# joaobuibergen/roms-trunk-mgh

Hardware: AMD Instinct MI355X
Metric: simulated-days/wall-sec (higher is better)
Workload: dtype f64; 1 GPU; BENCHMARK3 2048x256x30 NT=2 nonlinear 3-D step incl. 59 step2d calls, U3/C4 tracer advection, analytic atmospheric forcing, bulk fluxes + KPP + diagnostics every step; tiling=1x1, halo_transport=none, rccl_ranks=0, graph_exchanges=1, ndtfast=20, finite=True

## Files before the change

### include/roms_hip.h

```cpp
#ifndef ROMS_HIP_H
#define ROMS_HIP_H

#ifdef __cplusplus
extern "C" {
#endif

enum roms_kind {
  K_2D = 0, K_2D_T2, K_2D_T3, K_2D_NT,
  K_3DR, K_3DW, K_3DR_T2, K_3DW_T2, K_3DW_NAT, K_4DT, K_3DR_NT, K_3DW_T3
};

enum roms_field_id {
#define ROMS_FIELD(name, kind, owner) FID_##name,
#include "roms_fields.def"
#undef ROMS_FIELD
  FID_COUNT
};

typedef struct roms_fields {
#define ROMS_FIELD(name, kind, owner) double *name;
#include "roms_fields.def"
#undef ROMS_FIELD
} roms_fields_t;

// ... 127 lines not shown
int roms_hip_set_diagnostics(int nDIA, int ntsDIA, int ntstart, int nrrec);
int roms_hip_set_diags(const roms_step_idx_t *s);
int roms_hip_get_diagnostic(int dia_id, int itrc, int accumulated, double *host, long n_doubles);
int roms_hip_dia_index(int dia_id, int hdif, int rotated);
int roms_hip_set_floats(int Nfloats, const int *Ftype, const double *Tinfo, const double *Fz0,
                        const double *xcoord, const double *ycoord);
int roms_hip_floats_put(const double *track, long n_track, const int *bounded, long n_bounded);
int roms_hip_floats_get(double *track, long n_track, int *bounded, long n_bounded);
int roms_hip_step_floats(const roms_step_idx_t *s, double time, const int nfl[5]);
int roms_hip_set_tides(int NTC, int MTC, const double *Tperiod, const double *SSH_Tamp, const double *SSH_Tphase,
                       const double *UV_Tangle, const double *UV_Tphase, const double *UV_Tmajor, const double *UV_Tminor,
                       const double *angler, double tide_start, int ramp_tides, double dstart,
                       int add_fsobc, const double *zeta_base, int add_m2obc, const double *ubar_base,
                       const double *vbar_base);
int roms_hip_tides(double time);
int roms_hip_wvelocity(const roms_step_idx_t *s);
int roms_hip_diag(const roms_step_idx_t *s, double *out12);

int roms_hip_step2d_loop(roms_step_idx_t *s, int *indx1);

int roms_hip_graph_exchanges(int on);
int roms_hip_graph_exchanges_state(void);

int roms_hip_exchange(int field_id, int level);

typedef struct { int peer; int tag; long count; double *buf; } roms_halo_msg_t;
typedef int (*roms_halo_relay_fn)(void *user, int nsend, const roms_halo_msg_t *send,
                                  int nrecv, const roms_halo_msg_t *recv);
int roms_hip_set_halo_relay(roms_halo_relay_fn fn, void *user);
int roms_hip_halo_plan(const roms_bounds_t *b, int rank, int *out);

int roms_hip_timing_enable(int on);
double roms_hip_timing_last_ms(const char *entry);

int roms_hip_calib_stream(long n_doubles);

int roms_hip_check_guards(void);

#ifdef __cplusplus
}
#endif
#endif
```

### roms_trunk_mgh_amd/csrc/capi.hip

```cpp
#include "roms_dev.h"
#include <algorithm>
#include <map>
#include <vector>

RomsCtx g_ctx;

static const int k_field_kind[FID_COUNT] = {
#define ROMS_FIELD(name, kind, owner) kind,
#include "roms_fields.def"
#undef ROMS_FIELD
};
static const char *k_field_name[FID_COUNT] = {
#define ROMS_FIELD(name, kind, owner) #name,
#include "roms_fields.def"
#undef ROMS_FIELD
};

int roms_fail(const char *where, const char *what)
{
  g_ctx.last_error = std::string(where) + ": " + what;
  return 8;
}

long roms_field_count(int kind, const roms_bounds_t &b)
// ... 216 lines not shown
    (void)hipStreamDestroy(g_ctx.stream);
    g_ctx.stream = nullptr;
    g_ctx.devc = nullptr;
    return roms_fail("roms_hip_init", "hipMalloc of the constant block failed");
  }
  memset(&g_ctx.hostc, 0, sizeof(RomsDev));
  g_ctx.devc_dirty = true;
  g_ctx.inited = true;
  g_ctx.loopback = false;
  if (g_ctx.have_nccl_id) {
    if (ntileI * ntileJ == 1 && rank != 0) { roms_hip_finalize(); return roms_fail("roms_hip_init", "one tile: rank must be 0"); }
    int rc = halo_init();
    if (rc) { roms_hip_finalize(); return rc; }
    g_ctx.loopback = ntileI * ntileJ == 1;
  }
  return 0;
}

extern "C" int roms_hip_finalize(void)
{
  if (!g_ctx.inited) return 0;
  (void)hipStreamSynchronize(g_ctx.stream);
  (void)roms_hip_graph_exchanges(0);
  roms_rowm_release();
  snapshot_release();
  halo_finalize();
  diag_release();
  for (int i = 0; i < FID_COUNT; i++) {
    guarded_free(&g_ctx.dev[i], &g_ctx.dev_base[i]);
    g_ctx.host[i] = nullptr;
    g_ctx.count[i] = 0;
  }
  for (int q = 0; q < ROMS_NWS3; q++) guarded_free(&g_ctx.hostc.ws3[q], &g_ctx.ws3_base[q]);
  for (int q = 0; q < 32; q++) guarded_free(&g_ctx.hostc.ws2[q], &g_ctx.ws2_base[q]);
  sources_release();
  clima_release();
  avg_release();
  floats_release();
  tides_release();
  dia_release();
  if (g_ctx.devc) (void)hipFree(g_ctx.devc);
  g_ctx.devc = nullptr;
  if (g_ctx.stream) (void)hipStreamDestroy(g_ctx.stream);
  g_ctx.stream = nullptr;
  g_ctx.inited = false;
  g_ctx.have_bounds = g_ctx.have_params = false;
// ... 509 lines not shown
```

### roms_trunk_mgh_amd/csrc/halo.hip

```cpp
#include "roms_dev.h"
#include <dlfcn.h>
#include <vector>

typedef struct { char internal[128]; } rccl_uid_t;
typedef void *rccl_comm_t;
typedef int (*fn_getuid)(rccl_uid_t *);
typedef int (*fn_initrank)(rccl_comm_t *, int, rccl_uid_t, int);
typedef int (*fn_destroy)(rccl_comm_t);
typedef int (*fn_send)(const void *, size_t, int, int, rccl_comm_t, hipStream_t);
typedef int (*fn_recv)(void *, size_t, int, int, rccl_comm_t, hipStream_t);
typedef int (*fn_group)(void);
typedef int (*fn_allreduce)(const void *, void *, size_t, int, int, rccl_comm_t, hipStream_t);
typedef const char *(*fn_errstr)(int);
static struct {
  bool loaded = false;
  fn_getuid getuid = nullptr;
  fn_initrank initrank = nullptr;
  fn_destroy destroy = nullptr;
  fn_send send = nullptr;
  fn_recv recv = nullptr;
  fn_group gstart = nullptr, gend = nullptr;
  fn_allreduce allreduce = nullptr;
  fn_errstr errstr = nullptr;
} rccl;
// ... 133 lines not shown
  const int Lm = b.Lm;
  double *P = A + (long)k * nij;
  for (int m = 1; m <= b.NghostPoints; m++) P[I2(Lm + m, j)] = P[I2(m, j)];
  for (int m = 0; m <= 2; m++) P[I2(-m, j)] = P[I2(Lm - m, j)];
}

struct PeriodicArgs {
  double *A[8];
  int koff[8], jmin[8], jmax[8];
  int n, nktot, jlo;
};
__global__ void k_periodic_multi(const RomsDev *__restrict__ c, PeriodicArgs a)
{
  DEV_PROLOGUE(c)
  const int j = a.jlo + blockIdx.x * blockDim.x + threadIdx.x;
  const int kk = blockIdx.y;
  int f = 0;
  while (f + 1 < a.n && kk >= a.koff[f + 1]) f++;
  if (kk >= a.nktot || j < a.jmin[f] || j > a.jmax[f]) return;
  const int Lm = b.Lm;
  double *P = a.A[f] + (long)(kk - a.koff[f]) * nij;
  for (int m = 1; m <= b.NghostPoints; m++) P[I2(Lm + m, j)] = P[I2(m, j)];
  for (int m = 0; m <= 2; m++) P[I2(-m, j)] = P[I2(Lm - m, j)];
}

#define HALO_MAX_ITEMS 8
#define HALO_MAX_MSGS 8
struct PackArgs {
  double *A[HALO_MAX_ITEMS];
  int koff[HALO_MAX_ITEMS];
  int n, nktot, nmsg, unpack;
  int i0[HALO_MAX_MSGS], j0[HALO_MAX_MSGS], wi[HALO_MAX_MSGS], wj[HALO_MAX_MSGS];
  long off[HALO_MAX_MSGS];
  double *buf;
  int LBi, LBj;
  long ni, nij;
};
__global__ void k_pack_multi(const RomsDev *__restrict__, PackArgs a)
{
  const int LBi = a.LBi, LBj = a.LBj;
  const long ni = a.ni, nij = a.nij;
  const int m = blockIdx.z;
  const int wi = a.wi[m], cnt = wi * a.wj[m];
  const int r = blockIdx.x * blockDim.x + threadIdx.x;
  const int kk = blockIdx.y;
  if (r >= cnt) return;
// ... 72 lines not shown
    out[q++] = x.peer; out[q++] = x.tag; out[q++] = x.i0; out[q++] = x.wi; out[q++] = x.j0; out[q++] = x.wj;
  }
  for (int m = 0; m < p.nrecv; m++) {
    const HaloMsg &x = p.recv[m];
    out[q++] = x.peer; out[q++] = x.tag; out[q++] = x.i0; out[q++] = x.wi; out[q++] = x.j0; out[q++] = x.wj;
  }
  return 0;
}

static void ensure_neigh();

bool halo_rccl_capturable() { return g_ctx.nccl_comm != nullptr && g_relay == nullptr; }
int halo_reserve_buffers()
{
  ensure_neigh();
  if (!g_have_plan) { g_plan = make_plan(g_ctx.b, g_neigh); g_have_plan = true; }
  long smax = 0, rmax = 0;
  for (int m = 0; m < g_plan.nsend; m++) smax += (long)g_plan.send[m].wi * g_plan.send[m].wj;
  for (int m = 0; m < g_plan.nrecv; m++) rmax += (long)g_plan.recv[m].wi * g_plan.recv[m].wj;
  const long planes = (long)HALO_MAX_ITEMS * (g_ctx.b.N + 1);
  return ensure_buffers((size_t)((smax > rmax ? smax : rmax) * planes));
}

struct HaloItem { int gtype, nk; double *A; };

static int exchange_all(const HaloItem *items, int nitems)
{
  if (!g_have_plan) { g_plan = make_plan(g_ctx.b, g_neigh); g_have_plan = true; }
  const HaloPlan &pl = g_plan;
  if (pl.nsend == 0 && pl.nrecv == 0) return 0;
  long nktot = 0;
  for (int f = 0; f < nitems; f++) nktot += items[f].nk;
  PackArgs pa;
  pa.n = nitems; pa.nktot = (int)nktot;
  pa.LBi = g_ctx.b.LBi; pa.LBj = g_ctx.b.LBj;
  pa.ni = g_ctx.b.UBi - g_ctx.b.LBi + 1;
  pa.nij = pa.ni * (long)(g_ctx.b.UBj - g_ctx.b.LBj + 1);
  {
    int koff = 0;
    for (int f = 0; f < nitems; f++) { pa.A[f] = items[f].A; pa.koff[f] = koff; koff += items[f].nk; }
  }
  long soff[HALO_MAX_MSGS], roff[HALO_MAX_MSGS], stot = 0, rtot = 0;
  int smax = 1, rmax = 1;
  for (int m = 0; m < pl.nsend; m++) {
    soff[m] = stot;
    const int cnt = pl.send[m].wi * pl.send[m].wj;
    stot += nktot * cnt;
// ... 59 lines not shown
  return 0;
}

static void ensure_neigh()
{
  const roms_bounds_t &b = g_ctx.b;
  if (!g_have_neigh) {
    int v[12];
    roms_hip_tile_neighbors(g_ctx.rank, b.ntileI, b.ntileJ, b.NghostPoints, b.NghostPoints,
                            b.EWperiodic, b.NSperiodic, v);
    g_neigh = Neigh{v[0], v[1], v[2], v[3], v[4], v[5], v[6], v[7], v[8], v[9], v[10], v[11]};
    if (g_ctx.loopback && b.EWperiodic) {
      g_neigh.Wtile = g_neigh.Etile = g_ctx.rank;
      if (b.NghostPoints != 3) g_neigh.GrecvW = g_neigh.GsendE = b.NghostPoints + 1;
    }
    g_have_neigh = true;
  }
}

static int halo_run(const HaloItem *items, int nitems)
{
  const roms_bounds_t &b = g_ctx.b;
  if (nitems <= 0) return 0;
  if (b.ntileI * b.ntileJ == 1 && !g_ctx.loopback) {
    if (!b.EWperiodic) return 0;
    for (int f0 = 0; f0 < nitems; f0 += HALO_MAX_ITEMS) {
      PeriodicArgs pa;
      pa.n = nitems - f0 < HALO_MAX_ITEMS ? nitems - f0 : HALO_MAX_ITEMS;
      int nktot = 0, jlo = b.UBj, jhi = b.LBj;
      for (int f = 0; f < pa.n; f++) {
        const HaloItem &it = items[f0 + f];
        int jmin, jmax;
        if (b.NSperiodic) { jmin = b.Jstr; jmax = b.Jend; }
        else { jmin = (it.gtype == GT_R || it.gtype == GT_U) ? b.JstrR : b.Jstr; jmax = b.JendR; }
        pa.A[f] = it.A; pa.koff[f] = nktot; pa.jmin[f] = jmin; pa.jmax[f] = jmax;
        nktot += it.nk;
        jlo = jmin < jlo ? jmin : jlo;
        jhi = jmax > jhi ? jmax : jhi;
      }
      pa.nktot = nktot; pa.jlo = jlo;
      dim3 grid((jhi - jlo + 1 + 63) / 64, nktot);
      hipLaunchKernelGGL(k_periodic_multi, grid, dim3(64), 0, g_ctx.stream, g_ctx.devc, pa);
    }
    KERNEL_CHECK("k_periodic_multi");
    return 0;
  }
// ... 4 lines not shown
      hipLaunchKernelGGL(k_periodic_ew, grid, dim3(64), 0, g_ctx.stream, g_ctx.devc, items[f].A, items[f].nk, b.LBj, b.UBj);
    }
    KERNEL_CHECK("k_periodic_ew");
  }
  for (int f0 = 0; f0 < nitems; f0 += HALO_MAX_ITEMS) {
    const int n = nitems - f0 < HALO_MAX_ITEMS ? nitems - f0 : HALO_MAX_ITEMS;
    const int rc = exchange_all(items + f0, n);
    if (rc) return rc;
  }
  return 0;
}

static std::vector<HaloItem> g_batch;
static bool g_batching = false;
void halo_batch_begin() { g_batching = true; g_batch.clear(); }
int halo_batch_end()
{
  g_batching = false;
  const int rc = halo_run(g_batch.data(), (int)g_batch.size());
  g_batch.clear();
  return rc;
}

int halo_exchange3d(int gtype, int nk, double *A)
{
  const HaloItem it{gtype, nk, A};
  if (g_batching) { g_batch.push_back(it); return 0; }
  return halo_run(&it, 1);
}

int halo_exchange2d(int gtype, double *A, int) { return halo_exchange3d(gtype, 1, A); }

static double *g_coll = nullptr;
static size_t g_coll_doubles = 0;
static void coll_release()
{
  if (g_coll) (void)hipHostFree(g_coll);
  g_coll = nullptr;
  g_coll_doubles = 0;
}
int halo_allreduce_sum(double *A, long n)
{
  if (n <= 0) return 0;
  const int world = g_ctx.ntileI * g_ctx.ntileJ, me = g_ctx.rank;
  if (g_ctx.nccl_comm) {
    if (!rccl.allreduce) return roms_fail("collect", "RCCL symbol ncclAllReduce missing");
    RCCL_TRY(rccl.allreduce(A, A, (size_t)n, RCCL_FLOAT64, RCCL_SUM, (rccl_comm_t)g_ctx.nccl_comm, g_ctx.stream));
    return 0;
  }
// ... 45 lines not shown
```

### roms_trunk_mgh_amd/csrc/k_base.hip

```cpp
#include "roms_dev.h"

int roms_entry_check(const char *name);

int lbc_code(const roms_params_t &p, int sd, int v)
{
  if (p.lbc[sd][v]) return p.lbc[sd][v];
  return sd == LBS_WEST ? p.lbc_west : sd == LBS_EAST ? p.lbc_east : sd == LBS_SOUTH ? p.lbc_south : p.lbc_north;
}

int check_lbc()
{
  const roms_bounds_t &b = g_ctx.b;
  const roms_params_t &p = g_ctx.p;
  if (b.NSperiodic)
    return roms_fail("check_lbc", "N-S periodic grids are not implemented on this path");
  for (int sd = LBS_WEST; sd <= LBS_NORTH; sd++) {
    const bool periodic = (sd <= LBS_EAST) ? b.EWperiodic != 0 : b.NSperiodic != 0;
    for (int v = 0; v < LBV_COUNT; v++) {
      const int c = lbc_code(p, sd, v);
      if (periodic) {
        if (c != LBC_PERIODIC) return roms_fail("check_lbc", "a periodic direction needs LBC = Per on both of its sides");
        continue;
      }
      bool ok = c == LBC_CLOSED || c == LBC_GRADIENT || c == LBC_CLAMPED || c == LBC_RADIATION || c == LBC_RADIATION_NUDGING;
// ... 371 lines not shown
  a.T = g_ctx.dev[FID_vbar] + (long)(know - 1) * nij_host();
  a.ssh_only = g_ctx.hostc.tides.ssh_only;
  bc_acquire(a);
  a.dt2d = dt2d;
  return edge_bc(a);
}
int bc_v2d(int kout, const roms_step_idx_t *s)
{
  BcArgs a = bc_args(LBV_VBAR, g_ctx.dev[FID_vbar] + (long)(kout - 1) * nij_host(), 1);
  int know = kout; double dt2d = 0.0;
  if (s) bc_know(s, &know, &dt2d);
  else if (needs_know(a)) return roms_fail("bc_v2d", "this condition needs the barotropic time indices");
  a.Xold = g_ctx.dev[FID_vbar] + (long)(know - 1) * nij_host();
  a.D = g_ctx.dev[FID_vbar_bry];
  a.Zn = g_ctx.dev[FID_zeta] + (long)(kout - 1) * nij_host();
  a.Z = g_ctx.dev[FID_zeta] + (long)(know - 1) * nij_host();
  a.Zb = g_ctx.dev[FID_zeta_bry];
  a.T = g_ctx.dev[FID_ubar] + (long)(know - 1) * nij_host();
  a.ssh_only = g_ctx.hostc.tides.ssh_only;
  bc_acquire(a);
  a.dt2d = dt2d;
  return edge_bc(a);
}
int bc_u3d(int nout, int nstp)
{
  const long n3r = nij_host() * g_ctx.b.N;
  BcArgs a = bc_args(LBV_U, g_ctx.dev[FID_u] + (long)(nout - 1) * n3r, g_ctx.b.N);
  a.Xold = g_ctx.dev[FID_u] + (long)(nstp - 1) * n3r;
  a.D = g_ctx.dev[FID_u_bry];
  return edge_bc(a);
}
int bc_v3d(int nout, int nstp)
{
  const long n3r = nij_host() * g_ctx.b.N;
  BcArgs a = bc_args(LBV_V, g_ctx.dev[FID_v] + (long)(nout - 1) * n3r, g_ctx.b.N);
  a.Xold = g_ctx.dev[FID_v] + (long)(nstp - 1) * n3r;
  a.D = g_ctx.dev[FID_v_bry];
  return edge_bc(a);
}
int bc_t3d(int nout, int itrc, int nstp)
{
  const long n3r = nij_host() * g_ctx.b.N;
  BcArgs a = bc_args(LBV_T, g_ctx.dev[FID_t] + ((long)(nout - 1) + 3L * (itrc - 1)) * n3r, g_ctx.b.N);
  a.Xold = g_ctx.dev[FID_t] + ((long)(nstp - 1) + 3L * (itrc - 1)) * n3r;
  a.D = g_ctx.dev[FID_t_bry] + (long)(itrc - 1) * n3r;
  const int ic = g_ctx.hostc.clima.ic[itrc - 1];
  if (ic > 0) a.C = g_ctx.hostc.clima.Tnudgcof + (long)(ic - 1) * n3r;
  return edge_bc(a);
}
int bc_w3d(double *A)
{
  int rc = edge_bc(bc_args(-1, A, g_ctx.b.N + 1));
  if (rc) return rc;
  return halo_exchange3d(GT_R, g_ctx.b.N + 1, A);
}

__global__ void __launch_bounds__(BLK_X *BLK_Y)
k_set_massflux(const RomsDev *__restrict__ c, int nrhs)
{
  DEV_PROLOGUE(c)
  const Blk XB = xcd_block();
  const int i = b.IstrT + XB.x * BLK_X + threadIdx.x;
  const int j = b.JstrT + XB.y * BLK_Y + threadIdx.y;
  const int k = XB.z + 1;
  if (i > b.IendT || j > b.JendT) return;
  const gcd_t Hz = (gcd_t)(c->F.Hz);
  const gcd_t u = (gcd_t)(c->F.u + (long)(nrhs - 1) * n3r);
  const gcd_t v = (gcd_t)(c->F.v + (long)(nrhs - 1) * n3r);
  const double hz = Hz[I3(i, j, k)];
  if (i >= b.IstrP)
    GF(Huon)[I3(i, j, k)] = 0.5 * (hz + Hz[I3(i - 1, j, k)]) * u[I3(i, j, k)] * GF(on_u)[I2(i, j)];
  if (j >= b.JstrP)
    GF(Hvom)[I3(i, j, k)] = 0.5 * (hz + Hz[I3(i, j - 1, k)]) * v[I3(i, j, k)] * GF(om_v)[I2(i, j)];
}

extern "C" int roms_hip_set_massflux(const roms_step_idx_t *s)
{
  int rc = roms_entry_check("roms_hip_set_massflux");
  if (rc) return rc;
  ScopedTimer tm("set_massflux");
  const roms_bounds_t &b = g_ctx.b;
  dim3 grid = grid2d(b.IendT - b.IstrT + 1, b.JendT - b.JstrT + 1);
  grid.z = b.N;
  hipLaunchKernelGGL(k_set_massflux, grid, block2d(), 0, g_ctx.stream, g_ctx.devc, s->nrhs);
  KERNEL_CHECK("k_set_massflux");
  halo_batch_begin();
  halo_exchange3d(GT_U, b.N, g_ctx.dev[FID_Huon]);
  halo_exchange3d(GT_V, b.N, g_ctx.dev[FID_Hvom]);
  return halo_batch_end();
}

template <int NMAX>
__global__ void __launch_bounds__(BLK_X *BLK_Y)
k_omega(const RomsDev *__restrict__ c)
{
  DEV_PROLOGUE(c)
  const Blk XB = xcd_block();
  const int i = b.Istr + XB.x * BLK_X + threadIdx.x;
  const int j = b.Jstr + XB.y * BLK_Y + threadIdx.y;
  if (i > b.Iend || j > b.Jend) return;
  const gcd_t Huon = (gcd_t)(c->F.Huon);
  const gcd_t Hvom = (gcd_t)(c->F.Hvom);
  const gcd_t z_w = (gcd_t)(c->F.z_w);
  const gd_t W = (gd_t)(c->F.W);
  double w[NMAX + 1];
  w[0] = 0.0;
#pragma unroll
  for (int k = 1; k <= NMAX; k++) {
    if (k <= N) {
      w[k] = w[k - 1] - (Huon[I3(i + 1, j, k)] - Huon[I3(i, j, k)] +
                         Hvom[I3(i, j + 1, k)] - Hvom[I3(i, j, k)]);
    }
  }
  const double zw0 = z_w[I3W(i, j, 0)];
  double wN = 0.0;
#pragma unroll
  for (int k = 1; k <= NMAX; k++) if (k == N) wN = w[k];
  const double wrk = wN / (z_w[I3W(i, j, N)] - zw0);
  W[I3W(i, j, 0)] = 0.0;
#pragma unroll
  for (int k = 1; k <= NMAX; k++) {
    if (k < N) W[I3W(i, j, k)] = w[k] - wrk * (z_w[I3W(i, j, k)] - zw0);
  }
  W[I3W(i, j, N)] = 0.0;
}

__global__ void k_src_omega(const RomsDev *__restrict__ c)
{
  DEV_PROLOGUE(c)
  const int is = blockIdx.x * blockDim.x + threadIdx.x;
  if (is >= c->src.n || c->src.D[is] != 2) return;
  const int i = c->src.I[is], j = c->src.J[is];
  if (i < b.Istr || i > b.Iend || j < b.Jstr || j > b.Jend) return;
  if (c->src.wmap[I2(i, j)] != is + 1) return;
  const double *__restrict__ Huon = c->F.Huon, *__restrict__ Hvom = c->F.Hvom, *__restrict__ z_w = c->F.z_w;
  double *__restrict__ W = c->F.W;
  double w = 0.0;
  for (int k = 1; k <= N; k++) {
    w = w - (Huon[I3(i + 1, j, k)] - Huon[I3(i, j, k)] + Hvom[I3(i, j + 1, k)] - Hvom[I3(i, j, k)]) +
        c->src.Qsrc[is + (long)c->src.n * (k - 1)];
    W[I3W(i, j, k)] = w;
  }
  const double zw0 = z_w[I3W(i, j, 0)];
  const double wrk = w / (z_w[I3W(i, j, N)] - zw0);
  for (int k = N - 1; k >= 1; k--) W[I3W(i, j, k)] = W[I3W(i, j, k)] - wrk * (z_w[I3W(i, j, k)] - zw0);
  W[I3W(i, j, N)] = 0.0;
}

extern "C" int roms_hip_omega(const roms_step_idx_t *s)
{
  (void)s;
  int rc = roms_entry_check("roms_hip_omega");
  if (rc) return rc;
  if ((rc = check_lbc())) return rc;
  ScopedTimer tm("omega");
  const roms_bounds_t &b = g_ctx.b;
  dim3 grid = grid2d(b.Iend - b.Istr + 1, b.Jend - b.Jstr + 1);
  if (b.N <= 16) hipLaunchKernelGGL(k_omega<16>, grid, block2d(), 0, g_ctx.stream, g_ctx.devc);
  else if (b.N <= 32) hipLaunchKernelGGL(k_omega<32>, grid, block2d(), 0, g_ctx.stream, g_ctx.devc);
  else hipLaunchKernelGGL(k_omega<ROMS_MAXN>, grid, block2d(), 0, g_ctx.stream, g_ctx.devc);
  KERNEL_CHECK("k_omega");
  if ((g_ctx.p.point_sources & 2) && g_ctx.hostc.src.n > 0) {
    hipLaunchKernelGGL(k_src_omega, dim3((g_ctx.hostc.src.n + 63) / 64), dim3(64), 0, g_ctx.stream, g_ctx.devc);
    KERNEL_CHECK("k_src_omega");
  }
  return bc_w3d(g_ctx.dev[FID_W]);
}

__global__ void k_set_zeta(const RomsDev *__restrict__ c)
{
  DEV_PROLOGUE(c)
  const Blk XB = xcd_block();
  const int i = b.IstrR + XB.x * BLK_X + threadIdx.x;
  const int j = b.JstrR + XB.y * BLK_Y + threadIdx.y;
  if (i > b.IendR || j > b.JendR) return;
  const double z = GF(Zt_avg1)[I2(i, j)];
  GF(zeta)[I2(i, j)] = z;
  GF(zeta)[I2(i, j) + nij] = z;
}

extern "C" int roms_hip_set_zeta(const roms_step_idx_t *s)
{
  (void)s;
  int rc = roms_entry_check("roms_hip_set_zeta");
  if (rc) return rc;
  ScopedTimer tm("set_zeta");
  const roms_bounds_t &b = g_ctx.b;
  hipLaunchKernelGGL(k_set_zeta, grid2d(b.IendR - b.IstrR + 1, b.JendR - b.JstrR + 1), block2d(), 0,
                     g_ctx.stream, g_ctx.devc);
  KERNEL_CHECK("k_set_zeta");
  return halo_exchange3d(GT_R, 2, g_ctx.dev[FID_zeta]);
}

__global__ void __launch_bounds__(BLK_X *BLK_Y)
k_set_depth(const RomsDev *__restrict__ c)
{
  DEV_PROLOGUE(c)
  const Blk XB = xcd_block();
  const int i = b.IstrT + XB.x * BLK_X + threadIdx.x;
  const int j = b.JstrT + XB.y * BLK_Y + threadIdx.y;
  if (i > b.IendT || j > b.JendT) return;
  const roms_params_t &p = c->p;
  const double hc = p.hc;
  double hwater = GF(h)[I2(i, j)];
  if (p.wet_dry && hwater == 0.0) {
    hwater = 1.0E-14;
    GF(h)[I2(i, j)] = hwater;
  }
  const double zt = GF(Zt_avg1)[I2(i, j)];
  const gd_t z_w = (gd_t)(c->F.z_w);
  const gd_t z_r = (gd_t)(c->F.z_r);
  const gd_t Hz = (gd_t)(c->F.Hz);
  double zw_prev = -hwater;
// ... 48 lines not shown
```

### roms_trunk_mgh_amd/csrc/k_physics.hip

```cpp
#include "roms_dev.h"
#include <cmath>

int roms_entry_check(const char *name);

namespace {

__global__ void __launch_bounds__(BLK_X *BLK_Y)
k_set_vbc(const RomsDev *__restrict__ c, int nrhs)
{
  DEV_PROLOGUE(c)
  const roms_params_t &p = c->p;
  const int i = b.IstrR + blockIdx.x * BLK_X + threadIdx.x;
  const int j = b.JstrR + blockIdx.y * BLK_Y + threadIdx.y;
  if (i > b.IendR || j > b.JendR) return;
  const long a = I2(i, j);
  const int NT = b.NT;
  const gcd_t u = (gcd_t)(c->F.u + (long)(nrhs - 1) * n3r);
  const gcd_t v = (gcd_t)(c->F.v + (long)(nrhs - 1) * n3r);
  GF(stflx)[a] = GF(stflux)[a];
  GF(btflx)[a] = GF(btflux)[a];
  if (p.salinity && NT >= 2) {
    const gcd_t S = (gcd_t)(c->F.t + ((long)(nrhs - 1) + 3L * 1) * n3r);
    const double EmP = GF(stflux)[a + nij];
    GF(stflx)[a + nij] = EmP * S[a + (long)(N - 1) * nij];
// ... 743 lines not shown
}

extern "C" int roms_hip_lmd_vmix(const roms_step_idx_t *s)
{
  int rc = roms_entry_check("roms_hip_lmd_vmix");
  if (rc) return rc;
  if ((rc = check_lbc())) return rc;
  const roms_bounds_t &b = g_ctx.b;
  if (b.NAT < 2 || !g_ctx.p.salinity) return roms_fail("roms_hip_lmd_vmix", "built for the SALINITY set-up (NAT = 2)");
  const long nij = (long)(b.UBi - b.LBi + 1) * (b.UBj - b.LBj + 1);
  const long n3w = nij * (b.N + 1);
  {
    ScopedTimer tm("lmd_vmix");
    const double vonKar = 0.41, lmd_Cstar = 10.0, lmd_Cv = 1.25, lmd_Ric = 0.3, lmd_betaT = -0.2, lmd_cs = 98.96,
                 lmd_epsilon = 0.1;
    const double lmd_Cg = lmd_Cstar * vonKar * pow(lmd_cs * vonKar * lmd_epsilon, 1.0 / 3.0);
    const double Vtc = lmd_Cv * sqrt(-lmd_betaT) / (sqrt(lmd_cs * lmd_epsilon) * lmd_Ric * vonKar * vonKar);
    const dim3 grid = grid2d(b.Iend - b.Istr + 1, b.Jend - b.Jstr + 1);
    if (b.N <= 32) hipLaunchKernelGGL(k_lmd_vmix<32>, grid, block2d(), 0, g_ctx.stream, g_ctx.devc, s->nstp, lmd_Cg, Vtc);
    else if (b.N <= ROMS_MAXN) hipLaunchKernelGGL(k_lmd_vmix<ROMS_MAXN>, grid, block2d(), 0, g_ctx.stream, g_ctx.devc, s->nstp, lmd_Cg, Vtc);
    else return roms_fail("roms_hip_lmd_vmix", "N > 64 not instantiated");
    KERNEL_CHECK("k_lmd_vmix");
    const int nj = b.Jend - b.Jstr + 1, ni_ = b.Iend - b.Istr + 1;
    if (b.west_edge || b.east_edge)
      hipLaunchKernelGGL(k_lmd_edges, dim3((nj + 63) / 64, b.N + 1), dim3(64), 0, g_ctx.stream, g_ctx.devc, 0);
    if (b.south_edge || b.north_edge)
      hipLaunchKernelGGL(k_lmd_edges, dim3((ni_ + 63) / 64, b.N + 1), dim3(64), 0, g_ctx.stream, g_ctx.devc, 1);
    if ((b.south_edge || b.north_edge) && (b.west_edge || b.east_edge))
      hipLaunchKernelGGL(k_lmd_edges, dim3(1, b.N + 1), dim3(64), 0, g_ctx.stream, g_ctx.devc, 2);
    KERNEL_CHECK("k_lmd_edges");
  }
  if (!b.EWperiodic && (rc = bc_generic(LBV_ZETA, LBV_ZETA, g_ctx.dev[FID_hsbl], 1))) return rc;
  if ((rc = halo_exchange2d(GT_R, g_ctx.dev[FID_hsbl]))) return rc;
  if ((rc = bc_w3d(g_ctx.dev[FID_Akv]))) return rc;
  for (int it = 0; it < b.NAT; it++)
    if ((rc = bc_w3d(g_ctx.dev[FID_Akt] + (long)it * n3w))) return rc;
  return 0;
}
```

### roms_trunk_mgh_amd/csrc/roms_dev.h

```cpp
#pragma once
#include <hip/hip_runtime.h>
#include <cstdio>
#include <cstring>
#include <string>
#include "roms_hip.h"

#define ROMS_NWS3 10

struct RomsSrc {
  int n;
  int ltr[ROMS_MAXNT];
  const int *I, *J, *D;
  const double *Qbar;
  const double *Qsrc;
  const double *Tsrc;
  const int *umap, *vmap;
  const int *wmap;
  const int *cells;
  int ncell;
  double *save;
};

struct RomsClima {
  int m2, m3, nt;
// ... 198 lines not shown
  const bool ltr = S.ltr[itrc - 1] != 0;
  const int N = c->b.N;
  auto face = [&](int m, long cf, long ckf, long off, const double *__restrict__ H, double &Fv) {
    if (!m) return;
    const int is = m - 1;
    if (ltr) Fv = H[ckf] * S.Tsrc[is + (long)S.n * ((k - 1) + (long)N * (itrc - 1))];
    else if (PRE) Fv = 0.0;
    else if (c->p.masking) {
      const double r1 = c->F.rmask[cf], r0 = c->F.rmask[cf - off];
      if (r1 == 0.0 && r0 == 1.0) Fv = H[ckf] * T[ckf - off];
      else if (r1 == 1.0 && r0 == 0.0) Fv = H[ckf] * T[ckf];
    }
  };
  face(S.umap[c0], c0, ck, 1, c->F.Huon, FXi);
  face(S.umap[c0 + 1], c0 + 1, ck + 1, 1, c->F.Huon, FXip1);
  face(S.vmap[c0], c0, ck, ni, c->F.Hvom, FEj);
  face(S.vmap[c0 + ni], c0 + ni, ck + ni, ni, c->F.Hvom, FEjp1);
}

#define I2(i,j)    ((long)((i) - LBi) + (long)((j) - LBj) * ni)
#define I3(i,j,k)  (I2(i,j) + (long)((k) - 1) * nij)
#define I3W(i,j,k) (I2(i,j) + (long)(k) * nij)

enum { GT_R = 0, GT_U, GT_V, GT_P };

#define BLK_X 64
#define BLK_Y 4
static inline dim3 grid2d(int nx, int ny) {
  return dim3((unsigned)((nx + BLK_X - 1) / BLK_X), (unsigned)((ny + BLK_Y - 1) / BLK_Y), 1);
}
static inline dim3 block2d() { return dim3(BLK_X, BLK_Y, 1); }
#define TP (BLK_X + 4)
#define TJ (BLK_Y + 4)
__device__ __forceinline__ double d2x(const double *f, int a) { return f[a - 1] - 2.0 * f[a] + f[a + 1]; }
__device__ __forceinline__ double d2y(const double *f, int a) { return f[a - TP] - 2.0 * f[a] + f[a + TP]; }
struct TileLv { int bx, by, k0; bool valid; };
#ifdef __HIPCC__
__device__ __forceinline__ TileLv decode_tile_level(int nx, int ny, int nz)
{
  const int nbx = (nx + BLK_X - 1) / BLK_X, nby = (ny + BLK_Y - 1) / BLK_Y;
  const int B = blockIdx.x, xcd = B & 7, q = B >> 3;
  TileLv r;
  r.k0 = q % nz;
  const int tl = (q / nz) * 8 + xcd;
  r.valid = tl < nbx * nby;
  r.bx = tl % nbx;
// ... 19 lines not shown
    const int tl = t * 8 + xcd;
    r.valid = tl < nbx * nby;
    r.bx = tl % nbx;
    r.by = tl / nbx;
  } else {
    const int x0 = (xcd * nbx) >> 3, w = (((xcd + 1) * nbx) >> 3) - x0;
    r.bx = x0 + t % w;
    r.by = t / w;
    r.valid = r.by < nby;
  }
  return r;
}
#endif
static inline dim3 grid_tile_tracer(int nx, int ny, int ntr, int ty = BLK_Y) {
  const int nbx = (nx + BLK_X - 1) / BLK_X, nby = (ny + ty - 1) / ty;
  if (nbx < 8) return dim3((unsigned)(((nbx * nby + 7) / 8) * 8 * ntr), 1, 1);
  return dim3((unsigned)(8 * ((nbx + 7) / 8) * nby * ntr), 1, 1);
}

int halo_exchange2d(int gtype, double *A, int nfields_stride_unused = 0);
int halo_exchange3d(int gtype, int nk, double *A);
void halo_batch_begin();
int halo_batch_end();
int halo_allreduce_sum(double *A, long n);
void floats_release();
void tides_release();
int guarded_alloc(double **user, double **base, long n);
void guarded_free(double **user, double **base);
void dia_release();
bool dia_on();
int dia_check(const char *where);
int dia_rate(int nnew);
int dia_arrays(const char *name[4], const double *base[4], long count[4]);
int bc_zeta(int kout, const roms_step_idx_t *s);
int bc_u2d(int kout, const roms_step_idx_t *s);
int bc_v2d(int kout, const roms_step_idx_t *s);
int bc_u3d(int nout, int nstp);
int bc_v3d(int nout, int nstp);
int bc_t3d(int nout, int itrc, int nstp);
bool lbc2d_all_closed();
int lbc_code(const roms_params_t &p, int sd, int v);
int bc_w3d(double *A);
int bc_generic(int gtype_var, int lbv, double *A, int nk);
void snapshot_release();
void snapshot_forget(int field_id);
void diag_release();
// ... 9 lines not shown
```

### roms_trunk_mgh_amd/hip.py

```python
import ctypes as C
import os

import numpy as np

from . import abi

_HERE = os.path.dirname(os.path.abspath(__file__))
LIB_PATH = os.path.join(_HERE, "libroms_hip.so")
_LIB = None


def use_library(path):
    global LIB_PATH
    if _LIB is not None:
        raise RuntimeError("use_library() after the library was loaded")
    LIB_PATH = os.path.abspath(path)

ENTRIES = ["set_massflux", "rho_eos", "omega", "set_zeta", "set_depth", "rhs3d",
           "pre_step3d", "prsgrd", "t3dmix2", "rhs3d_tile", "uv3dmix2", "step2d",
           "step3d_uv", "step3d_t", "bulk_flux", "set_vbc", "lmd_vmix", "wvelocity", "ini_zeta", "ini_fields",
           "t3dmix4", "uv3dmix4", "gls_prestep", "gls_corstep", "wetdry", "set_avg", "set_diags"]

DECLARED_SYMBOLS = (
    ["roms_hip_init", "roms_hip_finalize", "roms_hip_get_unique_id", "roms_hip_set_bounds",
     "roms_hip_set_params", "roms_hip_register_field", "roms_hip_sync_to_device",
     "roms_hip_sync_to_host", "roms_hip_sync_all_to_device", "roms_hip_sync_all_to_host",
     "roms_hip_device_ptr", "roms_hip_device_synchronize", "roms_hip_last_error",
     "roms_hip_step2d_loop", "roms_hip_exchange", "roms_hip_timing_enable",
     "roms_hip_timing_last_ms", "roms_hip_calib_stream", "roms_hip_set_halo_relay", "roms_hip_diag",
     "roms_hip_snapshot_begin", "roms_hip_snapshot_end", "roms_hip_halo_plan",
     "roms_hip_ana_srflux", "roms_hip_check_guards", "roms_hip_row_metrics_state",
     "roms_hip_graph_exchanges", "roms_hip_graph_exchanges_state", "roms_hip_set_sources",
     "roms_hip_set_clima", "roms_hip_set_averages", "roms_hip_get_average", "roms_hip_average_device_ptr",
     "roms_hip_avg_phase", "roms_hip_set_floats", "roms_hip_floats_put", "roms_hip_floats_get",
     "roms_hip_step_floats", "roms_hip_set_tides", "roms_hip_tides", "roms_hip_set_diagnostics",
     "roms_hip_get_diagnostic", "roms_hip_dia_index"] + ["roms_hip_" + e for e in ENTRIES])


_DP = C.POINTER(C.c_double)
class HaloMsg(C.Structure):
    _fields_ = [("peer", C.c_int), ("tag", C.c_int), ("count", C.c_long), ("buf", _DP)]


RELAY_FN = C.CFUNCTYPE(C.c_int, C.c_void_p, C.c_int, C.POINTER(HaloMsg), C.c_int, C.POINTER(HaloMsg))


def load():
    global _LIB
    if _LIB is not None:
        return _LIB
    if not os.path.exists(LIB_PATH):
        raise RuntimeError(
            f"{LIB_PATH} not found: build it with `python -m roms_trunk_mgh_amd._build` "
            "(there is no CPU fallback for the HIP path)")
    lib = C.CDLL(LIB_PATH, mode=C.RTLD_GLOBAL)
# ... 234 lines not shown
                import sys
                print(f"halo relay failed: {e!r}", file=sys.stderr, flush=True)
                return 1
        self._relay = RELAY_FN(cb)
        self._chk(self.l.roms_hip_set_halo_relay(self._relay, None), "set_halo_relay")

    def calib_stream(self, n_doubles):
        self._chk(self.l.roms_hip_calib_stream(n_doubles), "calib_stream")

    def last_ms(self, entry):
        return self.l.roms_hip_timing_last_ms(entry.encode())

    def row_metrics_state(self):
        self.l.roms_hip_row_metrics_state.restype = C.c_int
        return int(self.l.roms_hip_row_metrics_state())

    def graph_exchanges(self, on=True):
        self._chk(self.l.roms_hip_graph_exchanges(int(on)), "graph_exchanges")

    def graph_exchanges_state(self):
        self.l.roms_hip_graph_exchanges_state.restype = C.c_int
        return int(self.l.roms_hip_graph_exchanges_state())

    def check_guards(self):
        self._chk(self.l.roms_hip_check_guards(), "check_guards")

    def close(self):
        if RomsHip._live is self:
            import sys
            import warnings
            RomsHip._live = None
            rc = self.l.roms_hip_check_guards()
            msg = self.l.roms_hip_last_error() if rc else None
            self.l.roms_hip_finalize()
            if rc:
                text = msg.decode() if msg else ""
                what = ("guard band damaged: " if "store outside" in text else "guard bands could not be checked: ") + text
                if sys.exc_info()[0] is not None:
                    warnings.warn("roms_hip: " + what)
                else:
                    raise RuntimeError("roms_hip: " + what)

    def __del__(self):
        try:
            self.close()
        except Exception:
# ... 2 lines not shown
```

Baseline: 0.2375 simulated-days/s.

## Fuse periodic halo and wall boundary updates into producer kernels for single-tile runs

For a single E-W periodic tile with closed N/S walls, set_massflux, omega and set_zeta now write the periodic ghost images and wall copies directly from the producing kernel through own_store, so the separate boundary and halo kernel launches are skipped. The KPP edge kernels and halo exchanges for Akv/Akt are replaced by one batched k_tail_multi kernel that applies wall and seam updates together. The goal is fewer small launches and fewer extra memory passes per step. In exchange the producer kernels do extra branchy stores, and correctness depends on the geometry guard and on the ghost-index mapping being right.

```diff
diff --git a/include/roms_hip.h b/include/roms_hip.h
--- a/include/roms_hip.h
+++ b/include/roms_hip.h
@@ -173,6 +173,9 @@
 int roms_hip_graph_exchanges(int on);
 int roms_hip_graph_exchanges_state(void);
 
+int roms_hip_edge_fusion(int on);
+int roms_hip_edge_fusion_state(void);
+
 int roms_hip_exchange(int field_id, int level);
 
 typedef struct { int peer; int tag; long count; double *buf; } roms_halo_msg_t;
diff --git a/roms_trunk_mgh_amd/csrc/capi.hip b/roms_trunk_mgh_amd/csrc/capi.hip
--- a/roms_trunk_mgh_amd/csrc/capi.hip
+++ b/roms_trunk_mgh_amd/csrc/capi.hip
@@ -262,6 +262,8 @@
   if (!g_ctx.inited) return 0;
   (void)hipStreamSynchronize(g_ctx.stream);
   (void)roms_hip_graph_exchanges(0);
+  (void)roms_hip_edge_fusion(1);
+  g_edge_fused_last = 0;
   roms_rowm_release();
   snapshot_release();
   halo_finalize();
diff --git a/roms_trunk_mgh_amd/csrc/halo.hip b/roms_trunk_mgh_amd/csrc/halo.hip
--- a/roms_trunk_mgh_amd/csrc/halo.hip
+++ b/roms_trunk_mgh_amd/csrc/halo.hip
@@ -179,6 +179,43 @@
   double *P = a.A[f] + (long)(kk - a.koff[f]) * nij;
   for (int m = 1; m <= b.NghostPoints; m++) P[I2(Lm + m, j)] = P[I2(m, j)];
   for (int m = 0; m <= 2; m++) P[I2(-m, j)] = P[I2(Lm - m, j)];
+}
+
+struct TailArgs {
+  double *A[8];
+  int koff[8];
+  unsigned char wall[8], ecol[8];
+  int n, nktot, nIpad;
+};
+__global__ void k_tail_multi(const RomsDev *__restrict__ c, TailArgs a)
+{
+  DEV_PROLOGUE(c)
+  const int kk = blockIdx.y;
+  int f = 0;
+  while (f + 1 < a.n && kk >= a.koff[f + 1]) f++;
+  if (kk >= a.nktot) return;
+  const bool wall = a.wall[f] != 0, ecol = a.ecol[f] != 0;
+  const int Lm = b.Lm;
+  const int js = b.Jstr - 1, jn = b.Jend + 1;
+  double *P = a.A[f] + (long)(kk - a.koff[f]) * nij;
+  auto value = [&](int i, int j) {
+    const int jr = !wall ? j : (j == js ? js + 1 : (j == jn ? jn - 1 : j));
+    const bool inner = jr >= b.Jstr && jr <= b.Jend;
+    return P[I2((ecol && inner && i == Lm - 1) ? Lm : i, jr)];
+  };
+  const int r = blockIdx.x * blockDim.x + threadIdx.x;
+  if (r < a.nIpad) {
+    const int i = b.Istr + r;
+    if (i > b.Iend || !wall) return;
+    P[I2(i, js)] = value(i, js);
+    P[I2(i, jn)] = value(i, jn);
+    return;
+  }
+  const int j = js + (r - a.nIpad);
+  if (j > jn) return;
+  if (ecol && j >= b.Jstr && j <= b.Jend) P[I2(Lm - 1, j)] = P[I2(Lm, j)];
+  for (int m = 1; m <= b.NghostPoints; m++) P[I2(Lm + m, j)] = value(m, j);
+  for (int m = 0; m <= 2; m++) P[I2(-m, j)] = value(Lm - m, j);
 }
 
 #define HALO_MAX_ITEMS 8
@@ -297,7 +334,7 @@
   return ensure_buffers((size_t)((smax > rmax ? smax : rmax) * planes));
 }
 
-struct HaloItem { int gtype, nk; double *A; };
+struct HaloItem { int gtype, nk; double *A; bool tail, ecol; };
 
 static int exchange_all(const HaloItem *items, int nitems)
 {
@@ -403,6 +440,29 @@
 {
   const roms_bounds_t &b = g_ctx.b;
   if (nitems <= 0) return 0;
+  bool any_tail = false;
+  for (int f = 0; f < nitems; f++) any_tail = any_tail || items[f].tail;
+  if (any_tail) {
+    if (!edge_fusion_geom()) return roms_fail("halo_tail3d", "the fused wall / seam update is built for one E-W periodic tile");
+    for (int f0 = 0; f0 < nitems; f0 += HALO_MAX_ITEMS) {
+      TailArgs ta;
+      ta.n = nitems - f0 < HALO_MAX_ITEMS ? nitems - f0 : HALO_MAX_ITEMS;
+      int nktot = 0;
+      for (int f = 0; f < ta.n; f++) {
+        const HaloItem &it = items[f0 + f];
+        if (it.gtype != GT_R) return roms_fail("halo_tail3d", "rho-type fields only");
+        ta.A[f] = it.A; ta.koff[f] = nktot; ta.wall[f] = it.tail; ta.ecol[f] = it.ecol;
+        nktot += it.nk;
+      }
+      ta.nktot = nktot;
+      ta.nIpad = (b.Iend - b.Istr + 1 + 63) / 64 * 64;
+      dim3 grid((ta.nIpad + b.Jend - b.Jstr + 3 + 63) / 64, nktot);
+      hipLaunchKernelGGL(k_tail_multi, grid, dim3(64), 0, g_ctx.stream, g_ctx.devc, ta);
+    }
+    KERNEL_CHECK("k_tail_multi");
+    g_edge_fused_last = 1;
+    return 0;
+  }
   if (b.ntileI * b.ntileJ == 1 && !g_ctx.loopback) {
     if (!b.EWperiodic) return 0;
     for (int f0 = 0; f0 < nitems; f0 += HALO_MAX_ITEMS) {
@@ -453,9 +513,16 @@
   return rc;
 }
 
+int halo_tail3d(int nk, double *A, bool ecol)
+{
+  const HaloItem it{GT_R, nk, A, true, ecol};
+  if (g_batching) { g_batch.push_back(it); return 0; }
+  return halo_run(&it, 1);
+}
+
 int halo_exchange3d(int gtype, int nk, double *A)
 {
-  const HaloItem it{gtype, nk, A};
+  const HaloItem it{gtype, nk, A, false, false};
   if (g_batching) { g_batch.push_back(it); return 0; }
   return halo_run(&it, 1);
 }
diff --git a/roms_trunk_mgh_amd/csrc/k_base.hip b/roms_trunk_mgh_amd/csrc/k_base.hip
--- a/roms_trunk_mgh_amd/csrc/k_base.hip
+++ b/roms_trunk_mgh_amd/csrc/k_base.hip
@@ -417,6 +417,15 @@
   a.dt2d = dt2d;
   return edge_bc(a);
 }
+int g_edge_fusion = 1;
+int g_edge_fused_last = 0;
+extern "C" int roms_hip_edge_fusion(int on)
+{
+  g_edge_fusion = on ? 1 : 0;
+  return 0;
+}
+extern "C" int roms_hip_edge_fusion_state(void) { return g_edge_fused_last; }
+
 int bc_u3d(int nout, int nstp)
 {
   const long n3r = nij_host() * g_ctx.b.N;
@@ -445,13 +454,14 @@
 }
 int bc_w3d(double *A)
 {
+  g_edge_fused_last = 0;
   int rc = edge_bc(bc_args(-1, A, g_ctx.b.N + 1));
   if (rc) return rc;
   return halo_exchange3d(GT_R, g_ctx.b.N + 1, A);
 }
 
 __global__ void __launch_bounds__(BLK_X *BLK_Y)
-k_set_massflux(const RomsDev *__restrict__ c, int nrhs)
+k_set_massflux(const RomsDev *__restrict__ c, int nrhs, int own)
 {
   DEV_PROLOGUE(c)
   const Blk XB = xcd_block();
@@ -463,10 +473,11 @@
   const gcd_t u = (gcd_t)(c->F.u + (long)(nrhs - 1) * n3r);
   const gcd_t v = (gcd_t)(c->F.v + (long)(nrhs - 1) * n3r);
   const double hz = Hz[I3(i, j, k)];
+  const OwnTargets ot = own_images(b, own, i);
   if (i >= b.IstrP)
-    GF(Huon)[I3(i, j, k)] = 0.5 * (hz + Hz[I3(i - 1, j, k)]) * u[I3(i, j, k)] * GF(on_u)[I2(i, j)];
+    own_store(GF(Huon), I3(i, j, k), 0.5 * (hz + Hz[I3(i - 1, j, k)]) * u[I3(i, j, k)] * GF(on_u)[I2(i, j)], ot, b.Lm);
   if (j >= b.JstrP)
-    GF(Hvom)[I3(i, j, k)] = 0.5 * (hz + Hz[I3(i, j - 1, k)]) * v[I3(i, j, k)] * GF(om_v)[I2(i, j)];
+    own_store(GF(Hvom), I3(i, j, k), 0.5 * (hz + Hz[I3(i, j - 1, k)]) * v[I3(i, j, k)] * GF(om_v)[I2(i, j)], ot, b.Lm);
 }
 
 extern "C" int roms_hip_set_massflux(const roms_step_idx_t *s)
@@ -477,8 +488,11 @@
   const roms_bounds_t &b = g_ctx.b;
   dim3 grid = grid2d(b.IendT - b.IstrT + 1, b.JendT - b.JstrT + 1);
   grid.z = b.N;
-  hipLaunchKernelGGL(k_set_massflux, grid, block2d(), 0, g_ctx.stream, g_ctx.devc, s->nrhs);
+  const int own = edge_fusion_geom();
+  hipLaunchKernelGGL(k_set_massflux, grid, block2d(), 0, g_ctx.stream, g_ctx.devc, s->nrhs, own);
   KERNEL_CHECK("k_set_massflux");
+  g_edge_fused_last = own;
+  if (own) return 0;
   halo_batch_begin();
   halo_exchange3d(GT_U, b.N, g_ctx.dev[FID_Huon]);
   halo_exchange3d(GT_V, b.N, g_ctx.dev[FID_Hvom]);
@@ -487,7 +501,7 @@
 
 template <int NMAX>
 __global__ void __launch_bounds__(BLK_X *BLK_Y)
-k_omega(const RomsDev *__restrict__ c)
+k_omega(const RomsDev *__restrict__ c, int own)
 {
   DEV_PROLOGUE(c)
   const Blk XB = xcd_block();
@@ -512,12 +526,13 @@
 #pragma unroll
   for (int k = 1; k <= NMAX; k++) if (k == N) wN = w[k];
   const double wrk = wN / (z_w[I3W(i, j, N)] - zw0);
-  W[I3W(i, j, 0)] = 0.0;
+  const OwnTargets ot = own_targets(b, own, i, j, ni);
+  own_store(W, I3W(i, j, 0), 0.0, ot, b.Lm);
 #pragma unroll
   for (int k = 1; k <= NMAX; k++) {
-    if (k < N) W[I3W(i, j, k)] = w[k] - wrk * (z_w[I3W(i, j, k)] - zw0);
-  }
-  W[I3W(i, j, N)] = 0.0;
+    if (k < N) own_store(W, I3W(i, j, k), w[k] - wrk * (z_w[I3W(i, j, k)] - zw0), ot, b.Lm);
+  }
+  own_store(W, I3W(i, j, N), 0.0, ot, b.Lm);
 }
 
 __global__ void k_src_omega(const RomsDev *__restrict__ c)
@@ -551,10 +566,13 @@
   ScopedTimer tm("omega");
   const roms_bounds_t &b = g_ctx.b;
   dim3 grid = grid2d(b.Iend - b.Istr + 1, b.Jend - b.Jstr + 1);
-  if (b.N <= 16) hipLaunchKernelGGL(k_omega<16>, grid, block2d(), 0, g_ctx.stream, g_ctx.devc);
-  else if (b.N <= 32) hipLaunchKernelGGL(k_omega<32>, grid, block2d(), 0, g_ctx.stream, g_ctx.devc);
-  else hipLaunchKernelGGL(k_omega<ROMS_MAXN>, grid, block2d(), 0, g_ctx.stream, g_ctx.devc);
+  const bool srcw = (g_ctx.p.point_sources & 2) && g_ctx.hostc.src.n > 0;
+  const int own = edge_fusion_geom() && !srcw;
+  if (b.N <= 16) hipLaunchKernelGGL(k_omega<16>, grid, block2d(), 0, g_ctx.stream, g_ctx.devc, own);
+  else if (b.N <= 32) hipLaunchKernelGGL(k_omega<32>, grid, block2d(), 0, g_ctx.stream, g_ctx.devc, own);
+  else hipLaunchKernelGGL(k_omega<ROMS_MAXN>, grid, block2d(), 0, g_ctx.stream, g_ctx.devc, own);
   KERNEL_CHECK("k_omega");
+  if (own) { g_edge_fused_last = 1; return 0; }
   if ((g_ctx.p.point_sources & 2) && g_ctx.hostc.src.n > 0) {
     hipLaunchKernelGGL(k_src_omega, dim3((g_ctx.hostc.src.n + 63) / 64), dim3(64), 0, g_ctx.stream, g_ctx.devc);
     KERNEL_CHECK("k_src_omega");
@@ -562,7 +580,7 @@
   return bc_w3d(g_ctx.dev[FID_W]);
 }
 
-__global__ void k_set_zeta(const RomsDev *__restrict__ c)
+__global__ void k_set_zeta(const RomsDev *__restrict__ c, int own)
 {
   DEV_PROLOGUE(c)
   const Blk XB = xcd_block();
@@ -570,8 +588,9 @@
   const int j = b.JstrR + XB.y * BLK_Y + threadIdx.y;
   if (i > b.IendR || j > b.JendR) return;
   const double z = GF(Zt_avg1)[I2(i, j)];
-  GF(zeta)[I2(i, j)] = z;
-  GF(zeta)[I2(i, j) + nij] = z;
+  const OwnTargets ot = own_images(b, own, i);
+  own_store(GF(zeta), I2(i, j), z, ot, b.Lm);
+  own_store(GF(zeta), I2(i, j) + nij, z, ot, b.Lm);
 }
 
 extern "C" int roms_hip_set_zeta(const roms_step_idx_t *s)
@@ -581,9 +600,12 @@
   if (rc) return rc;
   ScopedTimer tm("set_zeta");
   const roms_bounds_t &b = g_ctx.b;
+  const int own = edge_fusion_geom();
   hipLaunchKernelGGL(k_set_zeta, grid2d(b.IendR - b.IstrR + 1, b.JendR - b.JstrR + 1), block2d(), 0,
-                     g_ctx.stream, g_ctx.devc);
+                     g_ctx.stream, g_ctx.devc, own);
   KERNEL_CHECK("k_set_zeta");
+  g_edge_fused_last = own;
+  if (own) return 0;
   return halo_exchange3d(GT_R, 2, g_ctx.dev[FID_zeta]);
 }
 
diff --git a/roms_trunk_mgh_amd/csrc/k_physics.hip b/roms_trunk_mgh_amd/csrc/k_physics.hip
--- a/roms_trunk_mgh_amd/csrc/k_physics.hip
+++ b/roms_trunk_mgh_amd/csrc/k_physics.hip
@@ -789,13 +789,23 @@
     else return roms_fail("roms_hip_lmd_vmix", "N > 64 not instantiated");
     KERNEL_CHECK("k_lmd_vmix");
     const int nj = b.Jend - b.Jstr + 1, ni_ = b.Iend - b.Istr + 1;
-    if (b.west_edge || b.east_edge)
-      hipLaunchKernelGGL(k_lmd_edges, dim3((nj + 63) / 64, b.N + 1), dim3(64), 0, g_ctx.stream, g_ctx.devc, 0);
-    if (b.south_edge || b.north_edge)
-      hipLaunchKernelGGL(k_lmd_edges, dim3((ni_ + 63) / 64, b.N + 1), dim3(64), 0, g_ctx.stream, g_ctx.devc, 1);
-    if ((b.south_edge || b.north_edge) && (b.west_edge || b.east_edge))
-      hipLaunchKernelGGL(k_lmd_edges, dim3(1, b.N + 1), dim3(64), 0, g_ctx.stream, g_ctx.devc, 2);
-    KERNEL_CHECK("k_lmd_edges");
+    if (!edge_fusion_geom()) {
+      if (b.west_edge || b.east_edge)
+        hipLaunchKernelGGL(k_lmd_edges, dim3((nj + 63) / 64, b.N + 1), dim3(64), 0, g_ctx.stream, g_ctx.devc, 0);
+      if (b.south_edge || b.north_edge)
+        hipLaunchKernelGGL(k_lmd_edges, dim3((ni_ + 63) / 64, b.N + 1), dim3(64), 0, g_ctx.stream, g_ctx.devc, 1);
+      if ((b.south_edge || b.north_edge) && (b.west_edge || b.east_edge))
+        hipLaunchKernelGGL(k_lmd_edges, dim3(1, b.N + 1), dim3(64), 0, g_ctx.stream, g_ctx.devc, 2);
+      KERNEL_CHECK("k_lmd_edges");
+    }
+  }
+  if (edge_fusion_geom()) {
+    halo_batch_begin();
+    if ((rc = halo_exchange2d(GT_R, g_ctx.dev[FID_hsbl]))) return rc;
+    if ((rc = halo_tail3d(b.N + 1, g_ctx.dev[FID_Akv], true))) return rc;
+    for (int it = 0; it < b.NAT; it++)
+      if ((rc = halo_tail3d(b.N + 1, g_ctx.dev[FID_Akt] + (long)it * n3w, true))) return rc;
+    return halo_batch_end();
   }
   if (!b.EWperiodic && (rc = bc_generic(LBV_ZETA, LBV_ZETA, g_ctx.dev[FID_hsbl], 1))) return rc;
   if ((rc = halo_exchange2d(GT_R, g_ctx.dev[FID_hsbl]))) return rc;
diff --git a/roms_trunk_mgh_amd/csrc/roms_dev.h b/roms_trunk_mgh_amd/csrc/roms_dev.h
--- a/roms_trunk_mgh_amd/csrc/roms_dev.h
+++ b/roms_trunk_mgh_amd/csrc/roms_dev.h
@@ -244,6 +244,42 @@
 #define I3(i,j,k)  (I2(i,j) + (long)((k) - 1) * nij)
 #define I3W(i,j,k) (I2(i,j) + (long)(k) * nij)
 
+struct OwnTargets { bool e, w, any; long wall; };
+#ifdef __HIPCC__
+__device__ __forceinline__ OwnTargets own_targets(const roms_bounds_t &b, int on, int i, int j, long ni)
+{
+  OwnTargets t{false, false, false, 0};
+  if (!on) return t;
+  t.e = i <= b.NghostPoints;
+  t.w = i >= b.Lm - 2;
+  t.wall = j == b.Jstr ? -ni : 0;
+  if (j == b.Jend) t.wall = ni;
+  t.any = t.e || t.w || t.wall != 0;
+  return t;
+}
+__device__ __forceinline__ OwnTargets own_images(const roms_bounds_t &b, int on, int i)
+{
+  OwnTargets t{false, false, false, 0};
+  if (!on) return t;
+  t.e = i <= b.NghostPoints;
+  t.w = i >= b.Lm - 2;
+  t.any = t.e || t.w;
+  return t;
+}
+__device__ __forceinline__ void own_store(gd_t X, long q, double v, const OwnTargets &t, int Lm)
+{
+  X[q] = v;
+  if (!t.any) return;
+  if (t.e) X[q + Lm] = v;
+  if (t.w) X[q - Lm] = v;
+  if (t.wall != 0) {
+    X[q + t.wall] = v;
+    if (t.e) X[q + t.wall + Lm] = v;
+    if (t.w) X[q + t.wall - Lm] = v;
+  }
+}
+#endif
+
 enum { GT_R = 0, GT_U, GT_V, GT_P };
 
 #define BLK_X 64
@@ -309,6 +345,15 @@
 int halo_exchange3d(int gtype, int nk, double *A);
 void halo_batch_begin();
 int halo_batch_end();
+int halo_tail3d(int nk, double *A, bool ecol);
+extern int g_edge_fusion;
+extern int g_edge_fused_last;
+static inline bool edge_fusion_geom()
+{
+  const roms_bounds_t &b = g_ctx.b;
+  return g_edge_fusion && b.ntileI * b.ntileJ == 1 && !g_ctx.loopback && b.EWperiodic && !b.NSperiodic &&
+         b.south_edge && b.north_edge && b.east_edge && b.Lm >= 3 && b.Mm >= 2;
+}
 int halo_allreduce_sum(double *A, long n);
 void floats_release();
 void tides_release();
diff --git a/roms_trunk_mgh_amd/hip.py b/roms_trunk_mgh_amd/hip.py
--- a/roms_trunk_mgh_amd/hip.py
+++ b/roms_trunk_mgh_amd/hip.py
@@ -30,7 +30,8 @@
      "roms_hip_timing_last_ms", "roms_hip_calib_stream", "roms_hip_set_halo_relay", "roms_hip_diag",
      "roms_hip_snapshot_begin", "roms_hip_snapshot_end", "roms_hip_halo_plan",
      "roms_hip_ana_srflux", "roms_hip_check_guards", "roms_hip_row_metrics_state",
-     "roms_hip_graph_exchanges", "roms_hip_graph_exchanges_state", "roms_hip_set_sources",
+     "roms_hip_graph_exchanges", "roms_hip_graph_exchanges_state", "roms_hip_edge_fusion",
+     "roms_hip_edge_fusion_state", "roms_hip_set_sources",
      "roms_hip_set_clima", "roms_hip_set_averages", "roms_hip_get_average", "roms_hip_average_device_ptr",
      "roms_hip_avg_phase", "roms_hip_set_floats", "roms_hip_floats_put", "roms_hip_floats_get",
      "roms_hip_step_floats", "roms_hip_set_tides", "roms_hip_tides", "roms_hip_set_diagnostics",
@@ -311,6 +312,13 @@
         self.l.roms_hip_graph_exchanges_state.restype = C.c_int
         return int(self.l.roms_hip_graph_exchanges_state())
 
+    def edge_fusion(self, on=True):
+        self._chk(self.l.roms_hip_edge_fusion(int(on)), "edge_fusion")
+
+    def edge_fusion_state(self):
+        self.l.roms_hip_edge_fusion_state.restype = C.c_int
+        return int(self.l.roms_hip_edge_fusion_state())
+
     def check_guards(self):
         self._chk(self.l.roms_hip_check_guards(), "check_guards")
 
```

New measurement: 0.2401 simulated-days/s (median of 6 runs). 1.01x the previous value.
